# AgentMaker/PAPC

Measured on AMD Instinct MI355X. Metric: point-clouds/sec (fwd+bwd) PointNet++SSG B=32 N=4096, higher is better.
Workload: dtype f32

## Files before the change

papc_amd/csrc/capi.hip:

```cpp
#include <stdarg.h>
#include <string.h>

#include <mutex>
#include <vector>

#include "common.h"

#define GEMM_PARTS_DEFAULT 768

namespace papc {

static thread_local char g_err[512] = "";

void set_error(const char *fmt, ...)
{
    va_list ap;
    va_start(ap, fmt);
    vsnprintf(g_err, sizeof(g_err), fmt, ap);
    va_end(ap);
}

int check_launch(const char *what)
{
    hipError_t e = hipGetLastError();
// ... 17 lines not shown
    {"PAPC_GEMM_WS", 0, 0, 3},
    {"PAPC_GEMM_OCC", 0, 0, 1},
    {"PAPC_GEMM_DBG", 0, 0, 1},
    {"PAPC_GEMM_KB", 0, 0, 2},
    {"PAPC_GEMM_MINWG", 192, 1, 4096},
    {"PAPC_GEMM_TL", 0, 0, 1},
    {"PAPC_FPS_THREADS", 0, 0, 1024},
    {"PAPC_FPS_THREADS_SMALL", 0, 0, 1024},
    {"PAPC_STREAM", 1, 0, 1},
    {"PAPC_STREAM_MINTILES", 2048, 1, 1 << 30},
    {"PAPC_STREAM_CK", 0, 0, 8},
    {"PAPC_STREAM_ASM", 1, 0, 1},
    {"PAPC_PFN_MFMA", 1, 0, 1},
    {"PAPC_DW_RS64", 1, 0, 1},
    {"PAPC_DW_ROWS", 1, 0, 1},
    {"PAPC_DW_ROWS_BLOCKS", 4, 1, 16},
    {"PAPC_DW_ROWSX", 1, 0, 1},
    {"PAPC_PG_DBG", 0, 0, 15},
    {"PAPC_PG_NB", 0, 0, 2},
    {"PAPC_PG_NS", 0, 0, 3},
    {"PAPC_STREAM_MAXCAT", 1, 0, 1},
    {"PAPC_MAX_NOSTORE", 1, 0, 1},
    {"PAPC_PFN_FUSED_TAILS", 1, 0, 1},
    {"PAPC_STREAM_NW12", 1, 0, 1},
    {"PAPC_LG_LISTS", 1, 0, 1},
    {"PAPC_FOLD_WAVES", 16, 8, 16},
    {"PAPC_LGL_VARIANT", 0, 0, 3},
    {"PAPC_LG_PP", 1, 0, 1},
    {"PAPC_PG_GROUP", 1, 0, 1},
    {"PAPC_PG_PIPE", 1, 0, 1},
    {"PAPC_SEG_EPI", 1, 0, 1},
    {"PAPC_FOLD_FIN", 1, 0, 1},
    {"PAPC_XYZ1_RIDE", 1, 0, 1},
};
static int g_knobs[KNOB_COUNT];
static int knob_parse(int id, const char *e)
{
    const KnobDef &d = g_knob_defs[id];
    if (!e || !*e) return d.def;
    const int v = atoi(e);
    return (v < d.lo || v > d.hi) ? d.def : v;
}
static const bool g_knobs_loaded = [] {
    for (int i = 0; i < KNOB_COUNT; ++i) g_knobs[i] = knob_parse(i, getenv(g_knob_defs[i].name));
    return true;
}();
int knob(int id) { return g_knobs[id]; }

struct ProfState {
    std::mutex mu;
    unsigned mask = 0;
    std::vector<std::pair<hipEvent_t, hipEvent_t>> pending[PAPC_K_COUNT];
    std::vector<hipEvent_t> pool;
    double total_ms[PAPC_K_COUNT] = {0};
    int64_t launches[PAPC_K_COUNT] = {0};
};
static ProfState g_prof;

static hipEvent_t prof_get_event()
{
    if (!g_prof.pool.empty()) {
        hipEvent_t e = g_prof.pool.back();
        g_prof.pool.pop_back();
        return e;
    }
    hipEvent_t e;
// ... 140 lines not shown
```

papc_amd/csrc/common.h:

```cpp
#pragma once
#include <hip/hip_runtime.h>
#include <stdint.h>
#include <stdio.h>
#include <stdlib.h>
#include <string.h>
#include <algorithm>

#include "papc_hip.h"

namespace papc {

void set_error(const char *fmt, ...);
int check_launch(const char *what);

#define PAPC_REQUIRE(cond, code, ...)      \
    do {                                   \
        if (!(cond)) {                     \
            papc::set_error(__VA_ARGS__);  \
            return (code);                 \
        }                                  \
    } while (0)

enum Knob {
    KNOB_LG_PARTS, KNOB_DW_F32, KNOB_DW_DBG, KNOB_DW_XYZ, KNOB_PARTS, KNOB_GEMM_F32, KNOB_GEMM_WAVES, KNOB_MAXCAT_WAVES,
    KNOB_GEMM_WS, KNOB_GEMM_OCC, KNOB_GEMM_DBG, KNOB_GEMM_KB, KNOB_GEMM_MINWG, KNOB_GEMM_TL, KNOB_FPS_THREADS,
    KNOB_FPS_THREADS_SMALL, KNOB_STREAM, KNOB_STREAM_MINTILES, KNOB_STREAM_CK, KNOB_STREAM_ASM, KNOB_PFN_MFMA, KNOB_DW_RS64, KNOB_DW_ROWS, KNOB_DW_ROWS_BLOCKS, KNOB_DW_ROWSX, KNOB_PG_DBG, KNOB_PG_NB, KNOB_PG_NS, KNOB_STREAM_MAXCAT, KNOB_MAX_NOSTORE, KNOB_PFN_FUSED_TAILS, KNOB_STREAM_NW12, KNOB_LG_LISTS, KNOB_FOLD_WAVES, KNOB_LGL_VARIANT, KNOB_LG_PP, KNOB_PG_GROUP, KNOB_PG_PIPE, KNOB_SEG_EPI, KNOB_FOLD_FIN, KNOB_XYZ1_RIDE, KNOB_COUNT
};
int knob(int id);

struct ProfScope {
    int kernel;
    hipStream_t stream;
    bool on;
    hipEvent_t e0;
    ProfScope(int kernel, hipStream_t stream);
    ~ProfScope();
};

static inline hipStream_t as_stream(papc_stream_t s) { return reinterpret_cast<hipStream_t>(s); }

static inline int64_t cdiv(int64_t a, int64_t b) { return (a + b - 1) / b; }
static inline bool aligned16(const void *p) { return (reinterpret_cast<uintptr_t>(p) & 15) == 0; }

#define PAPC_DPP(v, ctrl, rmask) __builtin_amdgcn_update_dpp((int)(v), (int)(v), (ctrl), (rmask), 0xF, false)

__device__ __forceinline__ float wave_sum_f32_to_lane63(float v)
{
    float t;
    t = __int_as_float(PAPC_DPP(__float_as_int(v), 0xB1, 0xF));  v += t;
    t = __int_as_float(PAPC_DPP(__float_as_int(v), 0x4E, 0xF));  v += t;
    t = __int_as_float(PAPC_DPP(__float_as_int(v), 0x124, 0xF)); v += t;
    t = __int_as_float(PAPC_DPP(__float_as_int(v), 0x128, 0xF)); v += t;
    t = __int_as_float(__builtin_amdgcn_update_dpp(0, __float_as_int(v), 0x142, 0xA, 0xF, false)); v += t;
    t = __int_as_float(__builtin_amdgcn_update_dpp(0, __float_as_int(v), 0x143, 0xC, 0xF, false)); v += t;
    return v;
}

__device__ __forceinline__ float half_sum_f32(float v)
{
// ... 97 lines not shown
```

papc_amd/csrc/head.hip:

```cpp
#include "common.h"
#include "hashrng.h"

namespace papc {

typedef float f32x16 __attribute__((ext_vector_type(16)));

constexpr int HT = 512;
constexpr int HW = 8;
constexpr int HROWS_MAX = 256;
constexpr int TP = 33;
constexpr int HC_STAGE_FLOATS = 16384;

template <class T>
__device__ __forceinline__ void coh_st(T *p, T v) { __hip_atomic_store(p, v, __ATOMIC_RELAXED, __HIP_MEMORY_SCOPE_AGENT); }
template <class T>
__device__ __forceinline__ T coh_ld(const T *p) { return __hip_atomic_load(p, __ATOMIC_RELAXED, __HIP_MEMORY_SCOPE_AGENT); }
template <bool COH>
__device__ __forceinline__ float ld1(const float *p) { if constexpr (COH) return coh_ld(p); else return *p; }
template <bool COH>
__device__ __forceinline__ float4 ld4(const float *p)
{
    if constexpr (COH) return make_float4(coh_ld(p), coh_ld(p + 1), coh_ld(p + 2), coh_ld(p + 3));
    else return *reinterpret_cast<const float4 *>(p);
}
template <bool COH>
__device__ __forceinline__ void st1(float *p, float v) { if constexpr (COH) coh_st(p, v); else *p = v; }

__device__ __forceinline__ void grid_barrier(unsigned *bar, unsigned target)
{
    asm volatile("s_waitcnt vmcnt(0)" ::: "memory");
    __syncthreads();
    if (threadIdx.x == 0) {
        __hip_atomic_fetch_add(bar, 1u, __ATOMIC_RELAXED, __HIP_MEMORY_SCOPE_AGENT);
        while (__hip_atomic_load(bar, __ATOMIC_RELAXED, __HIP_MEMORY_SCOPE_AGENT) < target) __builtin_amdgcn_s_sleep(1);
// ... 49 lines not shown
{
    const int r = lane & 31, h = lane >> 5;
    const int gr = g_r0 + r, col = c0 + r;
    const bool g_ok = gr < g_rows, c_ok = col < ldw;
    const float *gp = G + (int64_t)(g_ok ? gr : 0) * Cn;
    const float *wp = Wn + (c_ok ? col : 0);
    const int nblk = (Cn + 7) >> 3;
    const int per = (nblk + HW - 1) / HW, blk_end = min(nblk, (wave + 1) * per);
    for (int blk0 = wave * per; blk0 < blk_end; blk0 += 2) {
        float4 a[2];
        float b[2][4];
#pragma unroll
        for (int j = 0; j < 2; ++j) {
            const int n = (blk0 + j < blk_end ? blk0 + j : nblk) * 8 + 4 * h;
            const int nc = n < Cn ? n : 0;
            a[j] = ld4<COH>(gp + nc);
#pragma unroll
            for (int i = 0; i < 4; ++i) b[j][i] = wp[(int64_t)(nc + i) * ldw];
        }
#pragma unroll
        for (int j = 0; j < 2; ++j) {
            const int n = (blk0 + j < blk_end ? blk0 + j : nblk) * 8 + 4 * h;
            const bool ok = n < Cn;
            const float4 av = (ok && g_ok) ? a[j] : make_float4(0.f, 0.f, 0.f, 0.f);
            const bool bk = ok && c_ok;
            acc = __builtin_amdgcn_mfma_f32_32x32x2f32(av.x, bk ? b[j][0] : 0.f, acc, 0, 0, 0);
            acc = __builtin_amdgcn_mfma_f32_32x32x2f32(av.y, bk ? b[j][1] : 0.f, acc, 0, 0, 0);
            acc = __builtin_amdgcn_mfma_f32_32x32x2f32(av.z, bk ? b[j][2] : 0.f, acc, 0, 0, 0);
            acc = __builtin_amdgcn_mfma_f32_32x32x2f32(av.w, bk ? b[j][3] : 0.f, acc, 0, 0, 0);
        }
    }
}

__device__ __forceinline__ void reduce_waves_to_tile(const f32x16 &acc, float *red, float *tile, int row0, int wave, int lane, int tid)
{
#pragma unroll
    for (int i = 0; i < 16; ++i) {
        const int row = (i & 3) + 8 * (i >> 2) + 4 * (lane >> 5);
        red[(wave * 32 + row) * TP + (lane & 31)] = acc[i];
    }
    __syncthreads();
    for (int e = tid; e < 1024; e += HT) {
        const int row = e >> 5, c = e & 31;
        float s = 0.f;
#pragma unroll
        for (int w = 0; w < HW; ++w) s += red[(w * 32 + row) * TP + c];
        tile[(row0 + row) * TP + c] = s;
    }
    __syncthreads();
}

struct HeadFwd {
    const float *x, *w, *bias, *gamma, *beta;
    int B, Cin, Cout, has_bn;
    float eps, momentum;
    float *running_mean, *running_var;
    int64_t *num_batches_tracked;
    float drop_p;
    const int64_t *rng_state;
    int layer_tag;
    int64_t *rng_bump;
    float *y, *mean, *invstd, *out;
    uint8_t *keep;
};

template <bool CIN, bool COUT>
__device__ __forceinline__ void head_fwd_body(const HeadFwd &a, const int bx)
{
    extern __shared__ float smem[];
    float *red = smem;
    float *tile = smem + HW * 32 * TP;
    __shared__ float s_mean[32], s_scale[32], s_shift[32];
    const int tid = threadIdx.x, wave = tid >> 6, lane = tid & 63;
    const int c0 = bx * 32;
    const int nrb = (a.B + 31) >> 5;
    const float *xin = a.x;
    bool staged = false;
    if constexpr (CIN) {
        const int Bpad0 = nrb * 32;
        if ((int64_t)a.B * a.Cin <= HC_STAGE_FLOATS) {
            float *xs = tile + Bpad0 * TP;
            const int n = a.B * a.Cin;
            for (int e = tid; e < n; e += HT) xs[e] = coh_ld(a.x + e);
            __syncthreads();
            xin = xs;
            staged = true;
        }
    }
    for (int rb = 0; rb < nrb; ++rb) {
        f32x16 acc = {0};
        if (CIN && !staged) mfma_kcontig<true>(acc, xin, a.B, rb * 32, a.w, a.Cout, c0, a.Cin, wave, lane);
        else mfma_kcontig<false>(acc, xin, a.B, rb * 32, a.w, a.Cout, c0, a.Cin, wave, lane);
        reduce_waves_to_tile(acc, red, tile, rb * 32, wave, lane, tid);
    }
    const int ncol = min(32, a.Cout - c0);
    {
        __shared__ float s_part[8][32];
        const int t = tid & 31, q = tid >> 5;
        const bool act = q < 8 && t < ncol;
        const float bv = (act && a.bias) ? a.bias[c0 + t] : 0.f;
        float sacc = 0.f;
        if (act) for (int b = q; b < a.B; b += 8) { const float v = tile[b * TP + t] + bv; tile[b * TP + t] = v; sacc += v; }
        if (q < 8) s_part[q][t] = sacc;
        __syncthreads();
        float mean = 0.f;
#pragma unroll
        for (int i = 0; i < 8; ++i) mean += s_part[i][t];
        mean /= (float)a.B;
        __syncthreads();
        float vacc = 0.f;
        if (act && a.has_bn == 1) for (int b = q; b < a.B; b += 8) { const float d = tile[b * TP + t] - mean; vacc += d * d; }
        if (q < 8) s_part[q][t] = vacc;
        __syncthreads();
        if (tid < ncol && a.has_bn == 1) {
            const int c = c0 + tid;
            float v = 0.f;
#pragma unroll
            for (int i = 0; i < 8; ++i) v += s_part[i][tid];
            const float var = v / (float)a.B;
            const float invstd = 1.0f / sqrtf(var + a.eps);
            a.mean[c] = mean;
            a.invstd[c] = invstd;
            if (a.running_mean) {
                a.running_mean[c] = (1.f - a.momentum) * a.running_mean[c] + a.momentum * mean;
                a.running_var[c] = (1.f - a.momentum) * a.running_var[c] + a.momentum * var;
            }
// ... 8 lines not shown
            if (a.mean) a.mean[c] = rm;
            if (a.invstd) a.invstd[c] = invstd;
            s_mean[tid] = rm;
            s_scale[tid] = invstd * a.gamma[c];
            s_shift[tid] = a.beta[c];
        }
        if (tid == 0 && bx == 0 && a.num_batches_tracked && a.has_bn == 1) a.num_batches_tracked[0] += 1;
    }
    __syncthreads();
    uint64_t seed = 0, counter = 0;
    const bool drop = a.rng_state != nullptr && a.drop_p > 0.f;
    if (drop) { seed = (uint64_t)a.rng_state[0]; counter = (uint64_t)a.rng_state[1]; }
    const float keep_scale = drop ? 1.0f / (1.0f - a.drop_p) : 1.0f;
    for (int e = tid; e < a.B * 32; e += HT) {
        const int b = e >> 5, t = e & 31;
        if (t >= ncol) continue;
        const int64_t o = (int64_t)b * a.Cout + c0 + t;
        const float yv = tile[b * TP + t];
        if (a.y) a.y[o] = yv;
        float v = yv;
        if (a.has_bn) {
            if (a.has_bn != 2) v = (yv - s_mean[t]) * s_scale[t] + s_shift[t];
            v = fmaxf(v, 0.f);
            bool k = true;
            if (drop) k = hash_uniform(seed, counter, (uint32_t)a.layer_tag, (uint32_t)o) >= a.drop_p;
            if (a.keep) a.keep[o] = k ? 1 : 0;
            v = k ? v * keep_scale : 0.f;
        }
        st1<COUT>(a.out + o, v);
    }
    if (a.rng_bump && bx == 0 && tid == 0) a.rng_bump[1] += 1;
}

__global__ __launch_bounds__(HT) void head_fwd_kernel(HeadFwd a) { head_fwd_body<false, false>(a, (int)blockIdx.x); }

struct HeadBwd {
    const float *gnext;
    const float *wnext;
    int Cn;
    const float *out, *y, *mean, *invstd, *gamma;
    float keep_scale;
    int has_bn;
    const float *x;
    int B, Cin, Cout;
    float *dy;
    float *dw, *db, *dgamma, *dbeta;
    int accumulate;
};

template <bool CIN, bool COUT>
__device__ __forceinline__ void head_bwd_body(const HeadBwd &a, const int bx, const int by, const int ny)
{
    extern __shared__ float smem[];
    float *red = smem;
    float *gt = smem + HW * 32 * TP;
    float *xh = gt + ((a.B + 31) & ~31) * TP;
    __shared__ float s_k1[32], s_k2[32], s_k3[32];
    const int tid = threadIdx.x, wave = tid >> 6, lane = tid & 63;
    const int c0 = bx * 32;
    const int nrb = (a.B + 31) >> 5;
    const int Bpad = nrb * 32;
    const int ncol = min(32, a.Cout - c0);
    if (a.wnext) {
        const float *gin = a.gnext;
        bool staged = false;
        if constexpr (CIN) {
            if ((int64_t)a.B * a.Cn <= HC_STAGE_FLOATS) {
                float *gs = xh + Bpad * TP;
                const int n = a.B * a.Cn;
                for (int e = tid; e < n; e += HT) gs[e] = coh_ld(a.gnext + e);
                __syncthreads();
                gin = gs;
                staged = true;
            }
        }
        for (int rb = 0; rb < nrb; ++rb) {
            f32x16 acc = {0};
            if (CIN && !staged) mfma_g_times_w<true>(acc, gin, a.B, rb * 32, a.wnext, a.Cn, a.Cout, c0, wave, lane);
            else mfma_g_times_w<false>(acc, gin, a.B, rb * 32, a.wnext, a.Cn, a.Cout, c0, wave, lane);
            reduce_waves_to_tile(acc, red, gt, rb * 32, wave, lane, tid);
        }
    } else {
        for (int e = tid; e < Bpad * 32; e += HT) {
            const int b = e >> 5, t = e & 31;
            gt[b * TP + t] = (b < a.B && t < ncol) ? ld1<CIN>(a.gnext + (int64_t)b * a.Cout + c0 + t) : 0.f;
        }
        __syncthreads();
    }
    if (a.has_bn == 2) {
        for (int e = tid; e < Bpad * 32; e += HT) {
            const int b = e >> 5, t = e & 31;
            float g = 0.f;
            if (b < a.B && t < ncol) g = a.out[(int64_t)b * a.Cout + c0 + t] > 0.f ? gt[b * TP + t] * a.keep_scale : 0.f;
            gt[b * TP + t] = g;
        }
        __syncthreads();
    } else if (a.has_bn) {
        for (int e = tid; e < Bpad * 32; e += HT) {
            const int b = e >> 5, t = e & 31;
            float g = 0.f, h = 0.f;
            if (b < a.B && t < ncol) {
                const int64_t o = (int64_t)b * a.Cout + c0 + t;
                g = a.out[o] > 0.f ? gt[b * TP + t] * a.keep_scale : 0.f;
                h = (a.y[o] - a.mean[c0 + t]) * a.invstd[c0 + t];
            }
            gt[b * TP + t] = g;
            xh[b * TP + t] = h;
        }
        __syncthreads();
        if (tid < 32) {
            float sg = 0.f, sgx = 0.f;
            for (int b = 0; b < a.B; ++b) { sg += gt[b * TP + tid]; sgx += gt[b * TP + tid] * xh[b * TP + tid]; }
            if (tid < ncol) {
                const int c = c0 + tid;
                if (by == 0) {
                    a.dbeta[c] = (a.accumulate ? a.dbeta[c] : 0.f) + sg;
                    a.dgamma[c] = (a.accumulate ? a.dgamma[c] : 0.f) + sgx;
                }
                s_k1[tid] = a.gamma[c] * a.invstd[c];
            } else {
                s_k1[tid] = 0.f;
            }
            s_k2[tid] = a.has_bn == 3 ? 0.f : sg / (float)a.B;
            s_k3[tid] = a.has_bn == 3 ? 0.f : sgx / (float)a.B;
        }
        __syncthreads();
        for (int e = tid; e < Bpad * 32; e += HT) {
            const int b = e >> 5, t = e & 31;
            float d = 0.f;
            if (b < a.B && t < ncol) d = s_k1[t] * ((gt[b * TP + t] - s_k2[t]) - xh[b * TP + t] * s_k3[t]);
            gt[b * TP + t] = d;
        }
        __syncthreads();
    }
    const bool first = by == 0;
    if (a.dy && first) {
        for (int e = tid; e < a.B * 32; e += HT) {
            const int b = e >> 5, t = e & 31;
            if (t < ncol) st1<COUT>(a.dy + (int64_t)b * a.Cout + c0 + t, gt[b * TP + t]);
        }
    }
    if (!a.x) return;
    if (first && tid < ncol && a.db) {
        float s = 0.f;
        for (int b = 0; b < a.B; ++b) s += gt[b * TP + tid];
        a.db[c0 + tid] = (a.accumulate ? a.db[c0 + tid] : 0.f) + s;
    }
    const int r = lane & 31, h = lane >> 5;
    for (int kb = by * HW + wave; kb * 32 < a.Cin; kb += HW * ny) {
        const int kcol = kb * 32 + r;
        const bool k_ok = kcol < a.Cin;
        const float *xp = a.x + (k_ok ? kcol : 0);
        f32x16 acc = {0};
        float prev[16];
#pragma unroll
        for (int i = 0; i < 16; ++i) {
            const int row = (i & 3) + 8 * (i >> 2) + 4 * h;
            prev[i] = (a.accumulate && row < ncol && k_ok) ? a.dw[(int64_t)(c0 + row) * a.Cin + kcol] : 0.f;
        }
        for (int b0 = 0; b0 < Bpad; b0 += 32) {
            float bv[16];
#pragma unroll
            for (int j = 0; j < 16; ++j) {
                const int b = b0 + 2 * j + h;
                bv[j] = xp[(int64_t)(b < a.B ? b : 0) * a.Cin];
            }
#pragma unroll
            for (int j = 0; j < 16; ++j) {
                const int b = b0 + 2 * j + h;
                const float av = gt[b * TP + r];
                acc = __builtin_amdgcn_mfma_f32_32x32x2f32(av, (k_ok && b < a.B) ? bv[j] : 0.f, acc, 0, 0, 0);
            }
        }
#pragma unroll
        for (int i = 0; i < 16; ++i) {
            const int row = (i & 3) + 8 * (i >> 2) + 4 * h;
            if (row < ncol && k_ok) a.dw[(int64_t)(c0 + row) * a.Cin + kcol] = prev[i] + acc[i];
        }
    }
}

__global__ __launch_bounds__(HT) void head_bwd_kernel(HeadBwd a) { head_bwd_body<false, false>(a, (int)blockIdx.x, (int)blockIdx.y, (int)gridDim.y); }

template <bool COH>
__device__ __forceinline__ void softmax_xent_body(const float *z, int ldz, const int64_t *__restrict__ label, int B, int C, float *__restrict__ loss,
                                                  float *__restrict__ dz, float *part )
{
    const int nt = blockDim.x;
    float acc = 0.f;
    for (int b = threadIdx.x; b < B; b += nt) {
        const float *row = z + (int64_t)b * ldz;
        float m = ld1<COH>(row);
        for (int c = 1; c < C; ++c) m = fmaxf(m, ld1<COH>(row + c));
        float s = 0.f;
        for (int c = 0; c < C; ++c) s += expf(ld1<COH>(row + c) - m);
        const float lse = m + logf(s);
        const int64_t y = label[b];
        if (y >= 0 && y < C) acc += lse - ld1<COH>(row + y);
        const float inv = 1.0f / (s * (float)B);
        for (int c = 0; c < C; ++c) {
            float g = expf(ld1<COH>(row + c) - m) * inv;
            if (c == y) g -= 1.0f / (float)B;
            dz[(int64_t)b * C + c] = g;
        }
    }
    part[threadIdx.x] = acc;
    __syncthreads();
    if (threadIdx.x == 0) {
        float t = 0.f;
        const int n = B < nt ? B : nt;
        for (int i = 0; i < n; ++i) t += part[i];
        loss[0] = t / (float)B;
    }
}

// ... 66 lines not shown
            if (bid == 0) softmax_xent_body<true>(a.out, a.Cout, c.labels, a.B, a.Cout, c.loss, c.dlogits, smem);
        }
    }
    if (c.n > 1 || (c.labels && c.l[c.n - 1].Cout > 32)) grid_exit(c.bar);
}

struct HeadChainBwd {
    HeadBwd j[HC_MAX];
    int gx[HC_MAX], gy[HC_MAX], off[HC_MAX], phase[HC_MAX];
    int n, n_phases;
    unsigned *bar;
};
__global__ __launch_bounds__(HT) void head_chain_bwd_kernel(HeadChainBwd c)
{
    const int bid = (int)blockIdx.x;
    for (int ph = 0; ph < c.n_phases; ++ph) {
        for (int j = 0; j < c.n; ++j) {
            if (c.phase[j] != ph) continue;
            const int local = bid - c.off[j];
            if (local >= 0 && local < c.gx[j] * c.gy[j]) {
                if (ph == 0) head_bwd_body<false, true>(c.j[j], local % c.gx[j], local / c.gx[j], c.gy[j]);
                else head_bwd_body<true, true>(c.j[j], local % c.gx[j], local / c.gx[j], c.gy[j]);
            }
        }
        if (ph < c.n_phases - 1) grid_barrier(c.bar, (unsigned)(ph + 1) * gridDim.x);
    }
    if (c.n_phases > 1) grid_exit(c.bar);
}

}

using namespace papc;

extern "C" {

int papc_head_fc_f32(const float *x, const float *w, const float *bias, const float *gamma, const float *beta, int B, int Cin, int Cout,
                     int has_bn, float eps, float momentum, float *running_mean, float *running_var, int64_t *num_batches_tracked,
                     float drop_p, const int64_t *rng_state, int layer_tag, int64_t *rng_bump, float *y, float *mean, float *invstd,
                     uint8_t *keep, float *out, papc_stream_t stream)
{
    PAPC_REQUIRE(x && w && out, PAPC_E_INVALID, "papc_head_fc_f32: null pointer");
    PAPC_REQUIRE(B >= 1 && B <= HROWS_MAX, PAPC_E_INVALID, "papc_head_fc_f32: B=%d not in [1, %d]", B, HROWS_MAX);
    PAPC_REQUIRE(Cin >= 4 && Cin % 4 == 0 && Cout >= 1, PAPC_E_INVALID, "papc_head_fc_f32: Cin=%d must be a multiple of 4", Cin);
    PAPC_REQUIRE(has_bn >= 0 && has_bn <= 3, PAPC_E_INVALID, "papc_head_fc_f32: has_bn=%d not in {0, 1, 2, 3}", has_bn);
    PAPC_REQUIRE(has_bn != 1 || (gamma && beta && mean && invstd && y), PAPC_E_INVALID, "papc_head_fc_f32: BatchNorm needs gamma/beta/mean/invstd/y");
    PAPC_REQUIRE(has_bn != 3 || (gamma && beta && running_mean && running_var), PAPC_E_INVALID, "papc_head_fc_f32: eval-mode BatchNorm needs gamma/beta/running_mean/running_var");
    PAPC_REQUIRE(drop_p >= 0.f && drop_p < 1.f, PAPC_E_INVALID, "papc_head_fc_f32: drop_p=%f", (double)drop_p);
    hipStream_t st = as_stream(stream);
    ProfScope prof(PAPC_K_MISC, st);
    HeadFwd a{x, w, bias, gamma, beta, B, Cin, Cout, has_bn, eps, momentum, running_mean, running_var, num_batches_tracked,
              drop_p, rng_state, layer_tag, rng_bump, y, mean, invstd, out, keep};
    const int Bpad = (B + 31) & ~31;
    const size_t lds = (size_t)(HW * 32 + Bpad) * TP * sizeof(float);
    if (lds > 48 * 1024 && hipFuncSetAttribute(reinterpret_cast<const void *>(head_fwd_kernel), hipFuncAttributeMaxDynamicSharedMemorySize, (int)lds) != hipSuccess)
        return check_launch("papc_head_fc_f32: hipFuncSetAttribute");
    hipLaunchKernelGGL(head_fwd_kernel, dim3((unsigned)cdiv(Cout, 32)), dim3(HT), lds, st, a);
    return check_launch("papc_head_fc_f32");
}

int papc_head_bwd_f32(const float *gnext, const float *wnext, int Cn, const float *out, const float *y, const float *mean,
                      const float *invstd, const float *gamma, float drop_p, int has_bn, const float *x, int B, int Cin, int Cout,
                      float *dy, float *dw, float *db, float *dgamma, float *dbeta, int accumulate, papc_stream_t stream)
{
    PAPC_REQUIRE(gnext, PAPC_E_INVALID, "papc_head_bwd_f32: null pointer");
    PAPC_REQUIRE(B >= 1 && B <= HROWS_MAX, PAPC_E_INVALID, "papc_head_bwd_f32: B=%d not in [1, %d]", B, HROWS_MAX);
    PAPC_REQUIRE(Cout >= 1 && (!wnext || (Cn >= 4 && Cn % 4 == 0)), PAPC_E_INVALID, "papc_head_bwd_f32: Cn=%d must be a multiple of 4", Cn);
    PAPC_REQUIRE(wnext || Cn == Cout, PAPC_E_INVALID, "papc_head_bwd_f32: without wnext, gnext must be [B, Cout]");
    PAPC_REQUIRE(has_bn >= 0 && has_bn <= 3, PAPC_E_INVALID, "papc_head_bwd_f32: has_bn=%d not in {0, 1, 2, 3}", has_bn);
    PAPC_REQUIRE((has_bn != 1 && has_bn != 3) || (out && y && mean && invstd && gamma && dgamma && dbeta), PAPC_E_INVALID, "papc_head_bwd_f32: BatchNorm backward needs the saved forward");
    PAPC_REQUIRE(has_bn != 2 || out, PAPC_E_INVALID, "papc_head_bwd_f32: ReLU backward needs the layer's output");
    PAPC_REQUIRE(!x || (dw && Cin >= 1), PAPC_E_INVALID, "papc_head_bwd_f32: x without dw");
    PAPC_REQUIRE(drop_p >= 0.f && drop_p < 1.f, PAPC_E_INVALID, "papc_head_bwd_f32: drop_p=%f", (double)drop_p);
    hipStream_t st = as_stream(stream);
    ProfScope prof(PAPC_K_MISC, st);
    HeadBwd a{gnext, wnext, Cn, out, y, mean, invstd, gamma, 1.0f / (1.0f - drop_p), has_bn, x, B, Cin, Cout, dy, dw, db, dgamma, dbeta, accumulate};
    const int Bpad = (B + 31) & ~31;
    const size_t lds = (size_t)(HW * 32 + 2 * Bpad) * TP * sizeof(float);
    if (lds > 48 * 1024 && hipFuncSetAttribute(reinterpret_cast<const void *>(head_bwd_kernel), hipFuncAttributeMaxDynamicSharedMemorySize, (int)lds) != hipSuccess)
        return check_launch("papc_head_bwd_f32: hipFuncSetAttribute");
    const int nsplit = x ? std::min(8, std::max(1, (int)cdiv(cdiv(Cin, 32), HW))) : 1;
    hipLaunchKernelGGL(head_bwd_kernel, dim3((unsigned)cdiv(Cout, 32), (unsigned)nsplit), dim3(HT), lds, st, a);
    return check_launch("papc_head_bwd_f32");
}

int papc_softmax_xent_f32(const float *logits, const int64_t *labels, int B, int C, float *loss, float *dlogits, papc_stream_t stream)
{
    PAPC_REQUIRE(logits && labels && loss && dlogits, PAPC_E_INVALID, "papc_softmax_xent_f32: null pointer");
    PAPC_REQUIRE(B >= 1 && C >= 1, PAPC_E_INVALID, "papc_softmax_xent_f32: B=%d C=%d", B, C);
    hipStream_t st = as_stream(stream);
    ProfScope prof(PAPC_K_MISC, st);
    if (B <= 1024) {
        hipLaunchKernelGGL(softmax_xent_kernel, dim3(1), dim3(256), 0, st, logits, labels, B, C, loss, dlogits);
    } else {
        if (hipMemsetAsync(loss, 0, sizeof(float), st) != hipSuccess) return check_launch("papc_softmax_xent_f32 (memset)");
        hipLaunchKernelGGL(softmax_xent_rows_kernel, dim3((unsigned)std::min(cdiv(B, 256), (int64_t)2048)), dim3(256), 0, st, logits, labels, B, C,
                           loss, dlogits);
    }
    return check_launch("papc_softmax_xent_f32");
}

int papc_head_chain_fwd_f32(const papc_head_fc_layer *layers, int n_layers, int B, const int64_t *rng_state, int64_t *rng_bump,
                            const int64_t *labels, float *loss, float *dlogits, uint32_t *sync, papc_stream_t stream)
{
    PAPC_REQUIRE(layers && sync, PAPC_E_INVALID, "papc_head_chain_fwd_f32: null pointer");
    PAPC_REQUIRE(n_layers >= 1 && n_layers <= HC_MAX, PAPC_E_UNSUPPORTED, "papc_head_chain_fwd_f32: %d layers (1..%d)", n_layers, HC_MAX);
    PAPC_REQUIRE(B >= 1 && B <= HROWS_MAX, PAPC_E_INVALID, "papc_head_chain_fwd_f32: B=%d not in [1, %d]", B, HROWS_MAX);
    PAPC_REQUIRE(!labels || (loss && dlogits), PAPC_E_INVALID, "papc_head_chain_fwd_f32: labels without loss / dlogits");
    HeadChainFwd c;
    memset(&c, 0, sizeof(c));
    int grid = 1;
    for (int i = 0; i < n_layers; ++i) {
        const papc_head_fc_layer &l = layers[i];
        PAPC_REQUIRE(l.x && l.w && l.out, PAPC_E_INVALID, "papc_head_chain_fwd_f32: layer %d: null pointer", i);
        PAPC_REQUIRE(l.Cin >= 4 && l.Cin % 4 == 0 && l.Cout >= 1, PAPC_E_INVALID, "papc_head_chain_fwd_f32: layer %d: Cin=%d must be a multiple of 4", i, l.Cin);
// ... 72 lines not shown
```

Baseline: 21970.

## Stage head FC GEMM operands through per-wave LDS with software prefetch

Adds a staged variant of the head fully-connected forward and backward kernels. Each wave loads coalesced float4 row pieces of both operands into a private padded LDS tile, prefetching the next sub-block while MFMAs run on the current one. The backward kernel also preloads BN, ReLU, bias and dW-accumulate operands into registers at kernel start to hide their latency. This costs more LDS per block and more registers, is selected by a new default-on knob, and falls back to the old path when LDS would exceed the cap.

```diff
diff --git a/papc_amd/csrc/capi.hip b/papc_amd/csrc/capi.hip
--- a/papc_amd/csrc/capi.hip
+++ b/papc_amd/csrc/capi.hip
@@ -73,6 +73,7 @@
     {"PAPC_SEG_EPI", 1, 0, 1},
     {"PAPC_FOLD_FIN", 1, 0, 1},
     {"PAPC_XYZ1_RIDE", 1, 0, 1},
+    {"PAPC_HEAD_STAGE", 1, 0, 1},
 };
 static int g_knobs[KNOB_COUNT];
 static int knob_parse(int id, const char *e)
diff --git a/papc_amd/csrc/common.h b/papc_amd/csrc/common.h
--- a/papc_amd/csrc/common.h
+++ b/papc_amd/csrc/common.h
@@ -24,7 +24,7 @@
 enum Knob {
     KNOB_LG_PARTS, KNOB_DW_F32, KNOB_DW_DBG, KNOB_DW_XYZ, KNOB_PARTS, KNOB_GEMM_F32, KNOB_GEMM_WAVES, KNOB_MAXCAT_WAVES,
     KNOB_GEMM_WS, KNOB_GEMM_OCC, KNOB_GEMM_DBG, KNOB_GEMM_KB, KNOB_GEMM_MINWG, KNOB_GEMM_TL, KNOB_FPS_THREADS,
-    KNOB_FPS_THREADS_SMALL, KNOB_STREAM, KNOB_STREAM_MINTILES, KNOB_STREAM_CK, KNOB_STREAM_ASM, KNOB_PFN_MFMA, KNOB_DW_RS64, KNOB_DW_ROWS, KNOB_DW_ROWS_BLOCKS, KNOB_DW_ROWSX, KNOB_PG_DBG, KNOB_PG_NB, KNOB_PG_NS, KNOB_STREAM_MAXCAT, KNOB_MAX_NOSTORE, KNOB_PFN_FUSED_TAILS, KNOB_STREAM_NW12, KNOB_LG_LISTS, KNOB_FOLD_WAVES, KNOB_LGL_VARIANT, KNOB_LG_PP, KNOB_PG_GROUP, KNOB_PG_PIPE, KNOB_SEG_EPI, KNOB_FOLD_FIN, KNOB_XYZ1_RIDE, KNOB_COUNT
+    KNOB_FPS_THREADS_SMALL, KNOB_STREAM, KNOB_STREAM_MINTILES, KNOB_STREAM_CK, KNOB_STREAM_ASM, KNOB_PFN_MFMA, KNOB_DW_RS64, KNOB_DW_ROWS, KNOB_DW_ROWS_BLOCKS, KNOB_DW_ROWSX, KNOB_PG_DBG, KNOB_PG_NB, KNOB_PG_NS, KNOB_STREAM_MAXCAT, KNOB_MAX_NOSTORE, KNOB_PFN_FUSED_TAILS, KNOB_STREAM_NW12, KNOB_LG_LISTS, KNOB_FOLD_WAVES, KNOB_LGL_VARIANT, KNOB_LG_PP, KNOB_PG_GROUP, KNOB_PG_PIPE, KNOB_SEG_EPI, KNOB_FOLD_FIN, KNOB_XYZ1_RIDE, KNOB_HEAD_STAGE, KNOB_COUNT
 };
 int knob(int id);
 
diff --git a/papc_amd/csrc/head.hip b/papc_amd/csrc/head.hip
--- a/papc_amd/csrc/head.hip
+++ b/papc_amd/csrc/head.hip
@@ -1,5 +1,6 @@
 #include "common.h"
 #include "hashrng.h"
+#include "head_stage.h"
 
 namespace papc {
 
@@ -115,19 +116,155 @@
     }
 }
 
-__device__ __forceinline__ void reduce_waves_to_tile(const f32x16 &acc, float *red, float *tile, int row0, int wave, int lane, int tid)
+constexpr int HSTG_WAVE = hstage::WAVE_FLOATS;
+constexpr size_t HSTG_LDS_MAX = 110 * 1024;
+
+struct StgRows { const float *p[hstage::LOADS]; };
+
+__device__ __forceinline__ StgRows stg_rows(const float *base, int rows, int r0, int K, int lane)
+{
+    StgRows s;
+#pragma unroll
+    for (int i = 0; i < hstage::LOADS; ++i) {
+        const int row = r0 + hstage::piece_row(i, lane);
+        s.p[i] = base + (int64_t)(row < rows ? row : rows - 1) * K;
+    }
+    return s;
+}
+__device__ __forceinline__ void stg_issue(float4 (&v)[hstage::LOADS], const StgRows &s, int K, const hstage::Range &rg, int t, int lane)
+{
+    const int k = hstage::piece_k(rg, t, lane);
+    const int kc = k < K ? k : 0;
+#pragma unroll
+    for (int i = 0; i < hstage::LOADS; ++i) v[i] = *reinterpret_cast<const float4 *>(s.p[i] + kc);
+}
+__device__ __forceinline__ void stg_write(float *tile, const float4 (&v)[hstage::LOADS], int rows, int r0, int K, const hstage::Range &rg, int t, int lane)
+{
+#pragma unroll
+    for (int i = 0; i < hstage::LOADS; ++i) {
+        const uint32_t m = hstage::piece_valid(rows, r0, K, rg, t, i, lane) ? 0xffffffffu : 0u;
+        *reinterpret_cast<float4 *>(tile + hstage::piece_lds(i, lane)) =
+            make_float4(__uint_as_float(__float_as_uint(v[i].x) & m), __uint_as_float(__float_as_uint(v[i].y) & m),
+                        __uint_as_float(__float_as_uint(v[i].z) & m), __uint_as_float(__float_as_uint(v[i].w) & m));
+    }
+}
+__device__ __forceinline__ void stg_frags(float4 (&f)[hstage::SUB], const float *tile, int lane)
+{
+#pragma unroll
+    for (int j = 0; j < hstage::SUB; ++j) f[j] = *reinterpret_cast<const float4 *>(tile + hstage::frag_lds(j, lane));
+}
+
+__device__ __forceinline__ int stg_wave() { return __builtin_amdgcn_readfirstlane((int)(threadIdx.x >> 6)); }
+
+__device__ __forceinline__ void mfma_kcontig_staged(f32x16 &acc, const float *__restrict__ A, int a_rows, int a_r0, const float *__restrict__ Bm,
+                                                    int b_rows, int b_r0, int K, int wave, int lane, float *stg)
+{
+    const hstage::Range rg = hstage::wave_range(K, wave);
+    const int T = hstage::sub_trips(rg);
+    if (T == 0) return;
+    float *ta = stg, *tb = stg + hstage::OP_FLOATS;
+    const StgRows ra = stg_rows(A, a_rows, a_r0, K, lane), rb = stg_rows(Bm, b_rows, b_r0, K, lane);
+    float4 va[hstage::LOADS], vb[hstage::LOADS];
+    stg_issue(va, ra, K, rg, 0, lane);
+    stg_issue(vb, rb, K, rg, 0, lane);
+    stg_write(ta, va, a_rows, a_r0, K, rg, 0, lane);
+    stg_write(tb, vb, b_rows, b_r0, K, rg, 0, lane);
+    for (int t = 0; t < T; ++t) {
+        const bool more = t + 1 < T;
+        if (more) {
+            stg_issue(va, ra, K, rg, t + 1, lane);
+            stg_issue(vb, rb, K, rg, t + 1, lane);
+        }
+        float4 fa[hstage::SUB], fb[hstage::SUB];
+        stg_frags(fa, ta, lane);
+        stg_frags(fb, tb, lane);
+        __builtin_amdgcn_sched_barrier(0);
+#pragma unroll
+        for (int j = 0; j < hstage::SUB; ++j) {
+            if (rg.blk0 + hstage::SUB * t + j < rg.blk_end) {
+                acc = __builtin_amdgcn_mfma_f32_32x32x2f32(fa[j].x, fb[j].x, acc, 0, 0, 0);
+                acc = __builtin_amdgcn_mfma_f32_32x32x2f32(fa[j].y, fb[j].y, acc, 0, 0, 0);
+                acc = __builtin_amdgcn_mfma_f32_32x32x2f32(fa[j].z, fb[j].z, acc, 0, 0, 0);
+                acc = __builtin_amdgcn_mfma_f32_32x32x2f32(fa[j].w, fb[j].w, acc, 0, 0, 0);
+            }
+        }
+        __builtin_amdgcn_sched_barrier(0);
+        if (more) {
+            stg_write(ta, va, a_rows, a_r0, K, rg, t + 1, lane);
+            stg_write(tb, vb, b_rows, b_r0, K, rg, t + 1, lane);
+        }
+    }
+}
+
+__device__ __forceinline__ void mfma_g_times_w_staged(f32x16 &acc, const float *__restrict__ G, int g_rows, int g_r0, const float *__restrict__ Wn,
+                                                      int Cn, int ldw, int c0, int wave, int lane, float *stg)
+{
+    const hstage::Range rg = hstage::wave_range(Cn, wave);
+    const int T = hstage::sub_trips(rg);
+    if (T == 0) return;
+    const int h = lane >> 5, col = c0 + (lane & 31);
+    const bool c_ok = col < ldw;
+    const float *wp = Wn + (c_ok ? col : 0);
+    const StgRows rgw = stg_rows(G, g_rows, g_r0, Cn, lane);
+    float4 va[hstage::LOADS];
+    float wn[hstage::SUB][4];
+    auto issue_w = [&](int t) {
+#pragma unroll
+        for (int j = 0; j < hstage::SUB; ++j) {
+            const int blk = rg.blk0 + hstage::SUB * t + j;
+            const int n = (blk < rg.blk_end ? blk : rg.nblk) * 8 + 4 * h;
+            const int nc = n < Cn ? n : 0;
+#pragma unroll
+            for (int i = 0; i < 4; ++i) wn[j][i] = wp[(int64_t)(nc + i) * ldw];
+        }
+    };
+    stg_issue(va, rgw, Cn, rg, 0, lane);
+    issue_w(0);
+    stg_write(stg, va, g_rows, g_r0, Cn, rg, 0, lane);
+    for (int t = 0; t < T; ++t) {
+        const bool more = t + 1 < T;
+        float b[hstage::SUB][4];
+#pragma unroll
+        for (int j = 0; j < hstage::SUB; ++j) {
+            const int blk = rg.blk0 + hstage::SUB * t + j;
+            const bool bk = blk < rg.blk_end && blk * 8 + 4 * h < Cn && c_ok;
+#pragma unroll
+            for (int i = 0; i < 4; ++i) b[j][i] = bk ? wn[j][i] : 0.f;
+        }
+        if (more) {
+            stg_issue(va, rgw, Cn, rg, t + 1, lane);
+            issue_w(t + 1);
+        }
+        float4 fa[hstage::SUB];
+        stg_frags(fa, stg, lane);
+        __builtin_amdgcn_sched_barrier(0);
+#pragma unroll
+        for (int j = 0; j < hstage::SUB; ++j) {
+            if (rg.blk0 + hstage::SUB * t + j < rg.blk_end) {
+                acc = __builtin_amdgcn_mfma_f32_32x32x2f32(fa[j].x, b[j][0], acc, 0, 0, 0);
+                acc = __builtin_amdgcn_mfma_f32_32x32x2f32(fa[j].y, b[j][1], acc, 0, 0, 0);
+                acc = __builtin_amdgcn_mfma_f32_32x32x2f32(fa[j].z, b[j][2], acc, 0, 0, 0);
+                acc = __builtin_amdgcn_mfma_f32_32x32x2f32(fa[j].w, b[j][3], acc, 0, 0, 0);
+            }
+        }
+        __builtin_amdgcn_sched_barrier(0);
+        if (more) stg_write(stg, va, g_rows, g_r0, Cn, rg, t + 1, lane);
+    }
+}
+
+__device__ __forceinline__ void reduce_waves_to_tile(const f32x16 &acc, float *red, int rstride, float *tile, int row0, int wave, int lane, int tid)
 {
 #pragma unroll
     for (int i = 0; i < 16; ++i) {
         const int row = (i & 3) + 8 * (i >> 2) + 4 * (lane >> 5);
-        red[(wave * 32 + row) * TP + (lane & 31)] = acc[i];
+        red[wave * rstride + row * TP + (lane & 31)] = acc[i];
     }
     __syncthreads();
     for (int e = tid; e < 1024; e += HT) {
         const int row = e >> 5, c = e & 31;
         float s = 0.f;
 #pragma unroll
-        for (int w = 0; w < HW; ++w) s += red[(w * 32 + row) * TP + c];
+        for (int w = 0; w < HW; ++w) s += red[w * rstride + row * TP + c];
         tile[(row0 + row) * TP + c] = s;
     }
     __syncthreads();
@@ -147,12 +284,14 @@
     uint8_t *keep;
 };
 
-template <bool CIN, bool COUT>
+template <bool CIN, bool COUT, bool STG = false>
 __device__ __forceinline__ void head_fwd_body(const HeadFwd &a, const int bx)
 {
+    static_assert(!(STG && CIN), "the chain flavours keep the unstaged loaders");
     extern __shared__ float smem[];
+    constexpr int RS = STG ? HSTG_WAVE : 32 * TP;
     float *red = smem;
-    float *tile = smem + HW * 32 * TP;
+    float *tile = smem + HW * RS;
     __shared__ float s_mean[32], s_scale[32], s_shift[32];
     const int tid = threadIdx.x, wave = tid >> 6, lane = tid & 63;
     const int c0 = bx * 32;
@@ -172,9 +311,10 @@
     }
     for (int rb = 0; rb < nrb; ++rb) {
         f32x16 acc = {0};
-        if (CIN && !staged) mfma_kcontig<true>(acc, xin, a.B, rb * 32, a.w, a.Cout, c0, a.Cin, wave, lane);
+        if constexpr (STG) mfma_kcontig_staged(acc, xin, a.B, rb * 32, a.w, a.Cout, c0, a.Cin, stg_wave(), lane, smem + stg_wave() * HSTG_WAVE);
+        else if (CIN && !staged) mfma_kcontig<true>(acc, xin, a.B, rb * 32, a.w, a.Cout, c0, a.Cin, wave, lane);
         else mfma_kcontig<false>(acc, xin, a.B, rb * 32, a.w, a.Cout, c0, a.Cin, wave, lane);
-        reduce_waves_to_tile(acc, red, tile, rb * 32, wave, lane, tid);
+        reduce_waves_to_tile(acc, red, RS, tile, rb * 32, wave, lane, tid);
     }
     const int ncol = min(32, a.Cout - c0);
     {
@@ -249,7 +389,8 @@
     if (a.rng_bump && bx == 0 && tid == 0) a.rng_bump[1] += 1;
 }
 
-__global__ __launch_bounds__(HT) void head_fwd_kernel(HeadFwd a) { head_fwd_body<false, false>(a, (int)blockIdx.x); }
+template <bool STG>
+__global__ __launch_bounds__(HT) void head_fwd_kernel(HeadFwd a) { head_fwd_body<false, false, STG>(a, (int)blockIdx.x); }
 
 struct HeadBwd {
     const float *gnext;
@@ -265,12 +406,14 @@
     int accumulate;
 };
 
-template <bool CIN, bool COUT>
+template <bool CIN, bool COUT, bool STG = false>
 __device__ __forceinline__ void head_bwd_body(const HeadBwd &a, const int bx, const int by, const int ny)
 {
+    static_assert(!(STG && CIN), "the chain flavours keep the unstaged loaders");
     extern __shared__ float smem[];
+    constexpr int RS = STG ? HSTG_WAVE : 32 * TP;
     float *red = smem;
-    float *gt = smem + HW * 32 * TP;
+    float *gt = smem + HW * RS;
     float *xh = gt + ((a.B + 31) & ~31) * TP;
     __shared__ float s_k1[32], s_k2[32], s_k3[32];
     const int tid = threadIdx.x, wave = tid >> 6, lane = tid & 63;
@@ -278,6 +421,48 @@
     const int nrb = (a.B + 31) >> 5;
     const int Bpad = nrb * 32;
     const int ncol = min(32, a.Cout - c0);
+    constexpr int NPRE = 2;
+    float p_out[NPRE] = {0.f, 0.f}, p_y[NPRE] = {0.f, 0.f}, p_mean = 0.f, p_invstd = 0.f, p_gamma = 0.f, p_dbeta = 0.f, p_dgamma = 0.f, p_db = 0.f;
+    float p_prev[16], p_x[16];
+    const int kb_first = by * HW + wave;
+    if constexpr (STG) {
+        if (a.has_bn) {
+            const int t = tid & 31;
+            const int tc = c0 + (t < ncol ? t : 0);
+#pragma unroll
+            for (int i = 0; i < NPRE; ++i) {
+                const int b = (tid + i * HT) >> 5;
+                const int64_t o = (int64_t)(b < a.B ? b : 0) * a.Cout + tc;
+                p_out[i] = a.out[o];
+                if (a.has_bn != 2) p_y[i] = a.y[o];
+            }
+            if (a.has_bn != 2) {
+                p_mean = a.mean[tc];
+                p_invstd = a.invstd[tc];
+                p_gamma = a.gamma[tc];
+                if (a.accumulate && by == 0 && tid < ncol) { p_dbeta = a.dbeta[tc]; p_dgamma = a.dgamma[tc]; }
+            }
+        }
+        if (a.x) {
+            if (a.accumulate && by == 0 && tid < ncol && a.db) p_db = a.db[c0 + tid];
+            if (kb_first * 32 < a.Cin) {
+                const int r = lane & 31, h = lane >> 5;
+                const int kcol = kb_first * 32 + r;
+                const bool k_ok = kcol < a.Cin;
+                const float *xp = a.x + (k_ok ? kcol : 0);
+#pragma unroll
+                for (int i = 0; i < 16; ++i) {
+                    const int row = (i & 3) + 8 * (i >> 2) + 4 * h;
+                    p_prev[i] = (a.accumulate && row < ncol && k_ok) ? a.dw[(int64_t)(c0 + row) * a.Cin + kcol] : 0.f;
+                }
+#pragma unroll
+                for (int j = 0; j < 16; ++j) {
+                    const int b = 2 * j + h;
+                    p_x[j] = xp[(int64_t)(b < a.B ? b : 0) * a.Cin];
+                }
+            }
+        }
+    }
     if (a.wnext) {
         const float *gin = a.gnext;
         bool staged = false;
@@ -293,9 +478,10 @@
         }
         for (int rb = 0; rb < nrb; ++rb) {
             f32x16 acc = {0};
-            if (CIN && !staged) mfma_g_times_w<true>(acc, gin, a.B, rb * 32, a.wnext, a.Cn, a.Cout, c0, wave, lane);
+            if constexpr (STG) mfma_g_times_w_staged(acc, gin, a.B, rb * 32, a.wnext, a.Cn, a.Cout, c0, stg_wave(), lane, smem + stg_wave() * HSTG_WAVE);
+            else if (CIN && !staged) mfma_g_times_w<true>(acc, gin, a.B, rb * 32, a.wnext, a.Cn, a.Cout, c0, wave, lane);
             else mfma_g_times_w<false>(acc, gin, a.B, rb * 32, a.wnext, a.Cn, a.Cout, c0, wave, lane);
-            reduce_waves_to_tile(acc, red, gt, rb * 32, wave, lane, tid);
+            reduce_waves_to_tile(acc, red, RS, gt, rb * 32, wave, lane, tid);
         }
     } else {
         for (int e = tid; e < Bpad * 32; e += HT) {
@@ -305,21 +491,26 @@
         __syncthreads();
     }
     if (a.has_bn == 2) {
-        for (int e = tid; e < Bpad * 32; e += HT) {
+        for (int i = 0, e = tid; e < Bpad * 32; ++i, e += HT) {
             const int b = e >> 5, t = e & 31;
             float g = 0.f;
-            if (b < a.B && t < ncol) g = a.out[(int64_t)b * a.Cout + c0 + t] > 0.f ? gt[b * TP + t] * a.keep_scale : 0.f;
+            if (b < a.B && t < ncol) {
+                const float ov = (STG && i == 0) ? p_out[0] : (STG && i == 1) ? p_out[1] : a.out[(int64_t)b * a.Cout + c0 + t];
+                g = ov > 0.f ? gt[b * TP + t] * a.keep_scale : 0.f;
+            }
             gt[b * TP + t] = g;
         }
         __syncthreads();
     } else if (a.has_bn) {
-        for (int e = tid; e < Bpad * 32; e += HT) {
+        for (int i = 0, e = tid; e < Bpad * 32; ++i, e += HT) {
             const int b = e >> 5, t = e & 31;
             float g = 0.f, h = 0.f;
             if (b < a.B && t < ncol) {
                 const int64_t o = (int64_t)b * a.Cout + c0 + t;
-                g = a.out[o] > 0.f ? gt[b * TP + t] * a.keep_scale : 0.f;
-                h = (a.y[o] - a.mean[c0 + t]) * a.invstd[c0 + t];
+                const float ov = (STG && i == 0) ? p_out[0] : (STG && i == 1) ? p_out[1] : a.out[o];
+                const float yv = (STG && i == 0) ? p_y[0] : (STG && i == 1) ? p_y[1] : a.y[o];
+                g = ov > 0.f ? gt[b * TP + t] * a.keep_scale : 0.f;
+                h = (yv - (STG ? p_mean : a.mean[c0 + t])) * (STG ? p_invstd : a.invstd[c0 + t]);
             }
             gt[b * TP + t] = g;
             xh[b * TP + t] = h;
@@ -331,10 +522,10 @@
             if (tid < ncol) {
                 const int c = c0 + tid;
                 if (by == 0) {
-                    a.dbeta[c] = (a.accumulate ? a.dbeta[c] : 0.f) + sg;
-                    a.dgamma[c] = (a.accumulate ? a.dgamma[c] : 0.f) + sgx;
+                    a.dbeta[c] = (a.accumulate ? (STG ? p_dbeta : a.dbeta[c]) : 0.f) + sg;
+                    a.dgamma[c] = (a.accumulate ? (STG ? p_dgamma : a.dgamma[c]) : 0.f) + sgx;
                 }
-                s_k1[tid] = a.gamma[c] * a.invstd[c];
+                s_k1[tid] = STG ? p_gamma * p_invstd : a.gamma[c] * a.invstd[c];
             } else {
                 s_k1[tid] = 0.f;
             }
@@ -361,7 +552,7 @@
     if (first && tid < ncol && a.db) {
         float s = 0.f;
         for (int b = 0; b < a.B; ++b) s += gt[b * TP + tid];
-        a.db[c0 + tid] = (a.accumulate ? a.db[c0 + tid] : 0.f) + s;
+        a.db[c0 + tid] = (a.accumulate ? (STG ? p_db : a.db[c0 + tid]) : 0.f) + s;
     }
     const int r = lane & 31, h = lane >> 5;
     for (int kb = by * HW + wave; kb * 32 < a.Cin; kb += HW * ny) {
@@ -370,17 +561,28 @@
         const float *xp = a.x + (k_ok ? kcol : 0);
         f32x16 acc = {0};
         float prev[16];
-#pragma unroll
-        for (int i = 0; i < 16; ++i) {
-            const int row = (i & 3) + 8 * (i >> 2) + 4 * h;
-            prev[i] = (a.accumulate && row < ncol && k_ok) ? a.dw[(int64_t)(c0 + row) * a.Cin + kcol] : 0.f;
+        const bool pre = STG && kb == kb_first;
+        if (pre) {
+#pragma unroll
+            for (int i = 0; i < 16; ++i) prev[i] = p_prev[i];
+        } else {
+#pragma unroll
+            for (int i = 0; i < 16; ++i) {
+                const int row = (i & 3) + 8 * (i >> 2) + 4 * h;
+                prev[i] = (a.accumulate && row < ncol && k_ok) ? a.dw[(int64_t)(c0 + row) * a.Cin + kcol] : 0.f;
+            }
         }
         for (int b0 = 0; b0 < Bpad; b0 += 32) {
             float bv[16];
-#pragma unroll
-            for (int j = 0; j < 16; ++j) {
-                const int b = b0 + 2 * j + h;
-                bv[j] = xp[(int64_t)(b < a.B ? b : 0) * a.Cin];
+            if (pre && b0 == 0) {
+#pragma unroll
+                for (int j = 0; j < 16; ++j) bv[j] = p_x[j];
+            } else {
+#pragma unroll
+                for (int j = 0; j < 16; ++j) {
+                    const int b = b0 + 2 * j + h;
+                    bv[j] = xp[(int64_t)(b < a.B ? b : 0) * a.Cin];
+                }
             }
 #pragma unroll
             for (int j = 0; j < 16; ++j) {
@@ -397,7 +599,8 @@
     }
 }
 
-__global__ __launch_bounds__(HT) void head_bwd_kernel(HeadBwd a) { head_bwd_body<false, false>(a, (int)blockIdx.x, (int)blockIdx.y, (int)gridDim.y); }
+template <bool STG>
+__global__ __launch_bounds__(HT) void head_bwd_kernel(HeadBwd a) { head_bwd_body<false, false, STG>(a, (int)blockIdx.x, (int)blockIdx.y, (int)gridDim.y); }
 
 template <bool COH>
 __device__ __forceinline__ void softmax_xent_body(const float *z, int ldz, const int64_t *__restrict__ label, int B, int C, float *__restrict__ loss,
@@ -530,6 +733,11 @@
 
 using namespace papc;
 
+static bool stg_lds_ok(const void *kernel)
+{
+    return hipFuncSetAttribute(kernel, hipFuncAttributeMaxDynamicSharedMemorySize, (int)HSTG_LDS_MAX) == hipSuccess;
+}
+
 extern "C" {
 
 int papc_head_fc_f32(const float *x, const float *w, const float *bias, const float *gamma, const float *beta, int B, int Cin, int Cout,
@@ -549,10 +757,16 @@
     HeadFwd a{x, w, bias, gamma, beta, B, Cin, Cout, has_bn, eps, momentum, running_mean, running_var, num_batches_tracked,
               drop_p, rng_state, layer_tag, rng_bump, y, mean, invstd, out, keep};
     const int Bpad = (B + 31) & ~31;
+    const size_t lds_stg = ((size_t)HW * HSTG_WAVE + (size_t)Bpad * TP) * sizeof(float);
+    if (knob(KNOB_HEAD_STAGE) && lds_stg <= HSTG_LDS_MAX) {
+        if (!stg_lds_ok(reinterpret_cast<const void *>(head_fwd_kernel<true>))) return check_launch("papc_head_fc_f32: hipFuncSetAttribute");
+        hipLaunchKernelGGL(head_fwd_kernel<true>, dim3((unsigned)cdiv(Cout, 32)), dim3(HT), lds_stg, st, a);
+        return check_launch("papc_head_fc_f32");
+    }
     const size_t lds = (size_t)(HW * 32 + Bpad) * TP * sizeof(float);
-    if (lds > 48 * 1024 && hipFuncSetAttribute(reinterpret_cast<const void *>(head_fwd_kernel), hipFuncAttributeMaxDynamicSharedMemorySize, (int)lds) != hipSuccess)
+    if (lds > 48 * 1024 && hipFuncSetAttribute(reinterpret_cast<const void *>(head_fwd_kernel<false>), hipFuncAttributeMaxDynamicSharedMemorySize, (int)lds) != hipSuccess)
         return check_launch("papc_head_fc_f32: hipFuncSetAttribute");
-    hipLaunchKernelGGL(head_fwd_kernel, dim3((unsigned)cdiv(Cout, 32)), dim3(HT), lds, st, a);
+    hipLaunchKernelGGL(head_fwd_kernel<false>, dim3((unsigned)cdiv(Cout, 32)), dim3(HT), lds, st, a);
     return check_launch("papc_head_fc_f32");
 }
 
@@ -573,11 +787,17 @@
     ProfScope prof(PAPC_K_MISC, st);
     HeadBwd a{gnext, wnext, Cn, out, y, mean, invstd, gamma, 1.0f / (1.0f - drop_p), has_bn, x, B, Cin, Cout, dy, dw, db, dgamma, dbeta, accumulate};
     const int Bpad = (B + 31) & ~31;
+    const int nsplit = x ? std::min(8, std::max(1, (int)cdiv(cdiv(Cin, 32), HW))) : 1;
+    const size_t lds_stg = ((size_t)HW * HSTG_WAVE + (size_t)2 * Bpad * TP) * sizeof(float);
+    if (knob(KNOB_HEAD_STAGE) && wnext && lds_stg <= HSTG_LDS_MAX) {
+        if (!stg_lds_ok(reinterpret_cast<const void *>(head_bwd_kernel<true>))) return check_launch("papc_head_bwd_f32: hipFuncSetAttribute");
+        hipLaunchKernelGGL(head_bwd_kernel<true>, dim3((unsigned)cdiv(Cout, 32), (unsigned)nsplit), dim3(HT), lds_stg, st, a);
+        return check_launch("papc_head_bwd_f32");
+    }
     const size_t lds = (size_t)(HW * 32 + 2 * Bpad) * TP * sizeof(float);
-    if (lds > 48 * 1024 && hipFuncSetAttribute(reinterpret_cast<const void *>(head_bwd_kernel), hipFuncAttributeMaxDynamicSharedMemorySize, (int)lds) != hipSuccess)
+    if (lds > 48 * 1024 && hipFuncSetAttribute(reinterpret_cast<const void *>(head_bwd_kernel<false>), hipFuncAttributeMaxDynamicSharedMemorySize, (int)lds) != hipSuccess)
         return check_launch("papc_head_bwd_f32: hipFuncSetAttribute");
-    const int nsplit = x ? std::min(8, std::max(1, (int)cdiv(cdiv(Cin, 32), HW))) : 1;
-    hipLaunchKernelGGL(head_bwd_kernel, dim3((unsigned)cdiv(Cout, 32), (unsigned)nsplit), dim3(HT), lds, st, a);
+    hipLaunchKernelGGL(head_bwd_kernel<false>, dim3((unsigned)cdiv(Cout, 32), (unsigned)nsplit), dim3(HT), lds, st, a);
     return check_launch("papc_head_bwd_f32");
 }
 
diff --git a/papc_amd/csrc/head_stage.h b/papc_amd/csrc/head_stage.h
--- /dev/null
+++ b/papc_amd/csrc/head_stage.h
@@ -0,0 +1,57 @@
+#pragma once
+#include <stdint.h>
+
+#if defined(__HIPCC__) || defined(__CUDACC__)
+#define PAPC_HD __host__ __device__ inline
+#else
+#define PAPC_HD inline
+#endif
+
+namespace papc {
+namespace hstage {
+
+constexpr int WAVES = 8;
+constexpr int SUB = 4;
+constexpr int LOADS = 4;
+constexpr int PITCH = 36;
+constexpr int OP_FLOATS = 32 * PITCH;
+constexpr int WAVE_FLOATS = 2 * OP_FLOATS;
+
+struct Range { int blk0, blk_end, nblk; };
+
+PAPC_HD Range wave_range(int K, int wave)
+{
+    const int nblk = (K + 7) >> 3;
+    const int per = (nblk + WAVES - 1) / WAVES;
+    const int end = (wave + 1) * per;
+    return Range{wave * per, end < nblk ? end : nblk, nblk};
+}
+PAPC_HD int sub_trips(const Range &rg) { return rg.blk_end > rg.blk0 ? (rg.blk_end - rg.blk0 + SUB - 1) / SUB : 0; }
+
+PAPC_HD int piece_row(int i, int lane) { return 8 * i + (lane >> 3); }
+PAPC_HD int piece_k(const Range &rg, int t, int lane) { return 8 * (rg.blk0 + SUB * t) + 4 * (lane & 7); }
+PAPC_HD bool piece_valid(int rows, int r0, int K, const Range &rg, int t, int i, int lane)
+{
+    const int blk = rg.blk0 + SUB * t + ((lane & 7) >> 1);
+    return r0 + piece_row(i, lane) < rows && blk < rg.blk_end && piece_k(rg, t, lane) < K;
+}
+PAPC_HD int64_t piece_goff(int rows, int r0, int K, const Range &rg, int t, int i, int lane)
+{
+    const int row = r0 + piece_row(i, lane);
+    const int k = piece_k(rg, t, lane);
+    return (int64_t)(row < rows ? row : rows - 1) * K + (k < K ? k : 0);
+}
+PAPC_HD int piece_lds(int i, int lane) { return piece_row(i, lane) * PITCH + 4 * (lane & 7); }
+
+PAPC_HD int frag_lds(int j, int lane) { return (lane & 31) * PITCH + 8 * j + 4 * (lane >> 5); }
+
+struct Frag { int row, k; bool valid; };
+PAPC_HD Frag parent_frag(int rows, int r0, int K, int blk, int lane)
+{
+    const int row = r0 + (lane & 31);
+    const int k = 8 * blk + 4 * (lane >> 5);
+    return Frag{row, k, row < rows && k < K};
+}
+
+}
+}
```

Result: no change. 21980 (median of 2 runs) (+0.0%).
